# Runnlion/gaussian-splatting-slam

Hardware: AMD Instinct MI355X
Metric: train_iters_per_sec (higher is better)
Workload: dtype f32

## Files before the change

gaussian-splatting-slam_amd/csrc/ssim.hip:

```cpp
#include "gsr_common.h"

#define ST 32
#ifndef SSIM_STY
#define SSIM_STY 16
#endif
#define STY SSIM_STY
#define SR 5
#define SH (ST + 2 * SR)
#define SHY (STY + 2 * SR)
#define RPT (STY / 8)

struct SsimWindow { float g[11]; };

static SsimWindow make_window() {
  SsimWindow w;
  double v[11], s = 0.0;
  for (int i = 0; i < 11; i++) { v[i] = exp(-(double)((i - 5) * (i - 5)) / (2.0 * 1.5 * 1.5)); s += v[i]; }
  float f[11], fs = 0.f;
  for (int i = 0; i < 11; i++) { f[i] = (float)v[i]; fs += f[i]; }
  for (int i = 0; i < 11; i++) w.g[i] = f[i] / fs;
  (void)s;
  return w;
}


#define SSIM_XCDS 8
#define NTRIP ((SHY * SH + 255) / 256)
#ifndef SSIM_FWD_WAVES
#define SSIM_FWD_WAVES 5
#endif
struct SsimTile { int x0, y0; size_t plane; };
struct SsimWalk { long long first; int count; };
__device__ __forceinline__ SsimWalk ssim_walk(int gx, int gy, int planes, int tpw) {
  const long long n = (long long)gx * gy * planes;
  const long long per = (n + SSIM_XCDS - 1) / SSIM_XCDS;
  const long long strip = blockIdx.x % SSIM_XCDS, off = (long long)(blockIdx.x / SSIM_XCDS) * tpw;
  SsimWalk w;
  w.first = strip * per + off;
  long long last = strip * per + (off + tpw < per ? off + tpw : per);
  if (last > n) last = n;
  w.count = last > w.first ? (int)(last - w.first) : 0;
  return w;
}
__device__ __forceinline__ SsimTile ssim_tile_at(long long lin, int gx, int gy, int H, int W) {
  const int plane = (int)(lin / ((long long)gx * gy));
  const int rem = (int)(lin - (long long)plane * gx * gy);
  const int ty = rem / gx;
  SsimTile t;
  t.x0 = (rem - ty * gx) * ST;
  t.y0 = ty * STY;
  t.plane = (size_t)plane * H * W;
  return t;
}
static inline unsigned ssim_grid(int gx, int gy, int planes, int tpw) {
  const long long n = (long long)gx * gy * planes;
  const long long per = (n + SSIM_XCDS - 1) / SSIM_XCDS;
  return (unsigned)(((per + tpw - 1) / tpw) * SSIM_XCDS);
}
static inline int ssim_fwd_tpw(int gx, int gy, int planes) {
  static const int forced = getenv("GSR_SSIM_TPW") ? atoi(getenv("GSR_SSIM_TPW")) : 0;
  if (forced > 0) return forced;
  return (long long)gx * gy * planes >= 4096 ? 2 : 1;
}

__global__ __launch_bounds__(256) __attribute__((amdgpu_waves_per_eu(SSIM_FWD_WAVES, SSIM_FWD_WAVES))) void k_ssim_fwd(int H, int W, int planes, float C1, float C2, SsimWindow win,
                                                  const float* __restrict__ img1, const float* __restrict__ img2,
                                                  float* __restrict__ ssim_map, float* __restrict__ dm_dmu1,
                                                  float* __restrict__ dm_dsigma1_sq, float* __restrict__ dm_dsigma12,
                                                  float* __restrict__ partials, int tpw) {
  __shared__ float sx[SHY][SH + 1], sy[SHY][SH + 1];
  __shared__ float hm[5][SHY][ST + 1];
  __shared__ float wsum[4][2];
  const int tid0 = threadIdx.x;
  const int gxn = (W + ST - 1) / ST, gyn = (H + STY - 1) / STY;
  const SsimWalk walk = ssim_walk(gxn, gyn, planes, tpw);
  if (walk.count <= 0) return;
  float ra[NTRIP], rb[NTRIP];
  auto fetch = [&](long long lin, int tid) {
    const SsimTile t = ssim_tile_at(lin, gxn, gyn, H, W);
    int r = tid / SH, c = tid - r * SH;
#pragma unroll
    for (int k = 0; k < NTRIP; k++) {
      const int gy = t.y0 + r - SR, gx = t.x0 + c - SR;
      float a = 0.f, b = 0.f;
      if (tid + 256 * k < SHY * SH && gy >= 0 && gy < H && gx >= 0 && gx < W) {
        a = (img1 + t.plane)[gy * W + gx];
        b = (img2 + t.plane)[gy * W + gx];
      }
      ra[k] = a;
      rb[k] = b;
      r += 256 / SH; c += 256 % SH;
      if (c >= SH) { c -= SH; r++; }
    }
  };
  fetch(walk.first, tid0);
  for (int ti = 0; ti < walk.count; ti++) {
    int tid = tid0;
    asm volatile("" : "+v"(tid));
    const long long lin = walk.first + ti;
    const SsimTile tile = ssim_tile_at(lin, gxn, gyn, H, W);
    const int x0 = tile.x0, y0 = tile.y0;
    const size_t plane = tile.plane;
    {
      int r = tid / SH, c = tid - r * SH;
#pragma unroll
      for (int k = 0; k < NTRIP; k++) {
        if (tid + 256 * k < SHY * SH) { sx[r][c] = ra[k]; sy[r][c] = rb[k]; }
        r += 256 / SH; c += 256 % SH;
        if (c >= SH) { c -= SH; r++; }
      }
    }
    __syncthreads();
    if (ti > 0 && tid == 0 && partials) {
      partials[2 * (size_t)(lin - 1)] = (wsum[0][0] + wsum[1][0]) + (wsum[2][0] + wsum[3][0]);
      partials[2 * (size_t)(lin - 1) + 1] = (wsum[0][1] + wsum[1][1]) + (wsum[2][1] + wsum[3][1]);
    }
    if (ti + 1 < walk.count) fetch(lin + 1, tid);
    float acc_ssim = 0.f, acc_l1 = 0.f;
    for (int i = tid; i < SHY * (ST / 4); i += 256) {
      const int r = i / (ST / 4), c0 = (i - r * (ST / 4)) * 4;
      float xa[14], ya[14];
#pragma unroll
      for (int k = 0; k < 14; k++) { xa[k] = sx[r][c0 + k]; ya[k] = sy[r][c0 + k]; }
      if (r >= SR && r < SR + STY && y0 + r - SR < H) {
#pragma unroll
        for (int j = 0; j < 4; j++)
          if (x0 + c0 + j < W) acc_l1 += fabsf(xa[SR + j] - ya[SR + j]);
      }
#pragma unroll
      for (int j = 0; j < 4; j++) {
        float m1 = 0.f, m2 = 0.f, s11 = 0.f, s22 = 0.f, s12 = 0.f;
#pragma unroll
        for (int k = 0; k < 11; k++) {
          const float w = win.g[k], a = xa[j + k], b = ya[j + k];
          m1 += w * a; m2 += w * b; s11 += w * a * a; s22 += w * b * b; s12 += w * a * b;
        }
        hm[0][r][c0 + j] = m1; hm[1][r][c0 + j] = m2; hm[2][r][c0 + j] = s11; hm[3][r][c0 + j] = s22; hm[4][r][c0 + j] = s12;
      }
    }
    __syncthreads();
    {
      const int c = tid & (ST - 1), r0 = (tid / ST) * RPT;
      float col[5][RPT + 10];
#pragma unroll
      for (int q = 0; q < 5; q++)
#pragma unroll
        for (int k = 0; k < RPT + 10; k++) col[q][k] = hm[q][r0 + k][c];
#pragma unroll
      for (int j = 0; j < RPT; j++) {
        const int r = r0 + j;
        const int gy = y0 + r, gx = x0 + c;
        if (gy >= H || gx >= W) continue;
        float mu1 = 0.f, mu2 = 0.f, e11 = 0.f, e22 = 0.f, e12 = 0.f;
#pragma unroll
        for (int k = 0; k < 11; k++) {
          const float w = win.g[k];
          mu1 += w * col[0][j + k]; mu2 += w * col[1][j + k]; e11 += w * col[2][j + k];
          e22 += w * col[3][j + k]; e12 += w * col[4][j + k];
        }
        const float mu1_sq = mu1 * mu1, mu2_sq = mu2 * mu2, mu12 = mu1 * mu2;
        const float sigma1_sq = e11 - mu1_sq, sigma2_sq = e22 - mu2_sq, sigma12 = e12 - mu12;
        const float A = 2.f * mu12 + C1, B = 2.f * sigma12 + C2;
        const float Cc = mu1_sq + mu2_sq + C1, D = sigma1_sq + sigma2_sq + C2;
        const float rCc = __builtin_amdgcn_rcpf(Cc), rD = __builtin_amdgcn_rcpf(D);
        const float inv = rCc * rD;
        const float m = A * B * inv;
        const size_t o = plane + (size_t)gy * W + gx;
        if (ssim_map) ssim_map[o] = m;
        acc_ssim += m;
        if (dm_dmu1) {
          dm_dmu1[o] = 2.f * mu2 * (B - A) * inv - m * 2.f * mu1 * rCc + m * 2.f * mu1 * rD;
          dm_dsigma1_sq[o] = -m * rD;
          dm_dsigma12[o] = 2.f * A * inv;
        }
      }
    }
    if (partials) {
#pragma unroll
      for (int sft = 32; sft > 0; sft >>= 1) {
        acc_ssim += __shfl_down(acc_ssim, sft, 64);
        acc_l1 += __shfl_down(acc_l1, sft, 64);
      }
      if ((tid & 63) == 0) { wsum[tid >> 6][0] = acc_ssim; wsum[tid >> 6][1] = acc_l1; }
    }
  }
  if (partials) {
    __syncthreads();
    if (tid0 == 0) {
      const size_t lin = (size_t)(walk.first + walk.count - 1);
      partials[2 * lin] = (wsum[0][0] + wsum[1][0]) + (wsum[2][0] + wsum[3][0]);
      partials[2 * lin + 1] = (wsum[0][1] + wsum[1][1]) + (wsum[2][1] + wsum[3][1]);
    }
  }
}

__global__ __launch_bounds__(256) void k_ssim_bwd(int H, int W, int planes, SsimWindow win, const float* __restrict__ img1,
                                                  const float* __restrict__ img2, const float* __restrict__ dL_dmap,
                                                  float g_const, float g_l1, const float* __restrict__ upstream,
                                                  const float* __restrict__ dm_dmu1,
                                                  const float* __restrict__ dm_dsigma1_sq,
                                                  const float* __restrict__ dm_dsigma12, float* __restrict__ dL_dimg1) {
  __shared__ float sa[3][SHY][SH + 1];
  const int tid = threadIdx.x;
  const int gxn = (W + ST - 1) / ST, gyn = (H + STY - 1) / STY;
  const SsimWalk walk = ssim_walk(gxn, gyn, planes, 1);
  if (walk.count <= 0) return;
  const SsimTile tile = ssim_tile_at(walk.first, gxn, gyn, H, W);
  const int x0 = tile.x0, y0 = tile.y0;
  const size_t plane = tile.plane;
  if (upstream) {
    const float u = upstream[0];
    g_const *= u;
    g_l1 *= u;
  }
  int lr = tid / SH, lc = tid - lr * SH;
  for (int i = tid; i < SHY * SH; i += 256) {
    const int r = lr, c = lc;
    lr += 256 / SH; lc += 256 % SH;
    if (lc >= SH) { lc -= SH; lr++; }
    const int gy = y0 + r - SR, gx = x0 + c - SR;
    float a = 0.f, b = 0.f, d = 0.f;
    if (gy >= 0 && gy < H && gx >= 0 && gx < W) {
      const size_t o = plane + (size_t)gy * W + gx;
      const float g = dL_dmap ? dL_dmap[o] : g_const;
      a = g * dm_dmu1[o];
      b = g * dm_dsigma1_sq[o];
      d = g * dm_dsigma12[o];
    }
    sa[0][r][c] = a; sa[1][r][c] = b; sa[2][r][c] = d;
  }
  __syncthreads();
  for (int i = tid; i < SHY * (ST / 4); i += 256) {
    const int r = i / (ST / 4), c0 = (i - r * (ST / 4)) * 4;
    float v0[14], v1[14], v2[14];
#pragma unroll
    for (int k = 0; k < 14; k++) { v0[k] = sa[0][r][c0 + k]; v1[k] = sa[1][r][c0 + k]; v2[k] = sa[2][r][c0 + k]; }
    asm volatile("" ::: "memory");
    __builtin_amdgcn_wave_barrier();
#pragma unroll
    for (int j = 0; j < 4; j++) {
      float t0 = 0.f, t1 = 0.f, t2 = 0.f;
#pragma unroll
      for (int k = 0; k < 11; k++) {
        const float w = win.g[k];
        t0 += w * v0[j + k]; t1 += w * v1[j + k]; t2 += w * v2[j + k];
      }
      sa[0][r][c0 + j] = t0; sa[1][r][c0 + j] = t1; sa[2][r][c0 + j] = t2;
    }
  }
  __syncthreads();
  {
    const int c = tid & (ST - 1), r0 = (tid / ST) * RPT;
    float col[3][RPT + 10];
#pragma unroll
    for (int q = 0; q < 3; q++)
#pragma unroll
      for (int k = 0; k < RPT + 10; k++) col[q][k] = sa[q][r0 + k][c];
#pragma unroll
    for (int j = 0; j < RPT; j++) {
      const int gy = y0 + r0 + j, gx = x0 + c;
      if (gy >= H || gx >= W) continue;
      float t0 = 0.f, t1 = 0.f, t2 = 0.f;
#pragma unroll
      for (int k = 0; k < 11; k++) {
        const float w = win.g[k];
        t0 += w * col[0][j + k]; t1 += w * col[1][j + k]; t2 += w * col[2][j + k];
      }
      const size_t o = plane + (size_t)gy * W + gx;
      const float x = img1[o], y = img2[o];
      float out = t0 + 2.f * x * t1 + y * t2;
      if (!dL_dmap) out += g_l1 * ((x > y) ? 1.f : ((x < y) ? -1.f : 0.f));
      dL_dimg1[o] = out;
    }
  }
}

extern "C" {

int gsr_fused_ssim_forward(int32_t planes, int32_t H, int32_t W, float C1, float C2, const float* img1,
                           const float* img2, float* ssim_map, float* dm_dmu1, float* dm_dsigma1_sq,
                           float* dm_dsigma12, void* stream) {
  if (planes < 0 || H <= 0 || W <= 0 || !img1 || !img2 || !ssim_map ||
      ((dm_dmu1 != nullptr) != (dm_dsigma1_sq != nullptr)) || ((dm_dmu1 != nullptr) != (dm_dsigma12 != nullptr))) {
    gsr_set_error("fused_ssim_forward: bad arguments");
    return GSR_ERR_INVALID_ARGUMENT;
  }
  if (planes == 0) return 0;
  static const SsimWindow win = make_window();
  hipStream_t st = (hipStream_t)stream;
  dim3 grid((W + ST - 1) / ST, (H + STY - 1) / STY, planes);
  const int tpw = ssim_fwd_tpw(grid.x, grid.y, planes);
  GSR_LAUNCH("ssim_fwd", k_ssim_fwd, dim3(ssim_grid(grid.x, grid.y, planes, tpw)), dim3(256), 0, st, H, W, planes, C1, C2, win, img1, img2,
             ssim_map, dm_dmu1, dm_dsigma1_sq, dm_dsigma12, (float*)nullptr, tpw);
  return gsr_launch_status("ssim forward launch");
}

int64_t gsr_fused_loss_blocks(int32_t planes, int32_t H, int32_t W) {
  return (int64_t)((W + ST - 1) / ST) * ((H + STY - 1) / STY) * planes;
}

#define LOSS_FIN_THREADS 1024
__global__ __launch_bounds__(LOSS_FIN_THREADS) void k_loss_finalize(const float* __restrict__ partials, long long nblk,
                                                                    float lambda, float inv_n, float* __restrict__ loss) {
  __shared__ float red[2][LOSS_FIN_THREADS / 64];
  const float2* pairs = reinterpret_cast<const float2*>(partials);
  float a = 0.f, b = 0.f;
  long long i = threadIdx.x;
  for (; i + 3 * LOSS_FIN_THREADS < nblk; i += 4 * LOSS_FIN_THREADS) {
    const float2 v0 = pairs[i], v1 = pairs[i + LOSS_FIN_THREADS], v2 = pairs[i + 2 * LOSS_FIN_THREADS],
                 v3 = pairs[i + 3 * LOSS_FIN_THREADS];
    a += v0.x; b += v0.y;
    a += v1.x; b += v1.y;
    a += v2.x; b += v2.y;
    a += v3.x; b += v3.y;
  }
  for (; i < nblk; i += LOSS_FIN_THREADS) {
    const float2 v = pairs[i];
    a += v.x;
    b += v.y;
  }
#pragma unroll
  for (int sft = 32; sft > 0; sft >>= 1) {
    a += __shfl_down(a, sft, 64);
    b += __shfl_down(b, sft, 64);
  }
  if ((threadIdx.x & 63) == 0) { red[0][threadIdx.x >> 6] = a; red[1][threadIdx.x >> 6] = b; }
  __syncthreads();
  if (threadIdx.x < 64) {
    a = threadIdx.x < LOSS_FIN_THREADS / 64 ? red[0][threadIdx.x] : 0.f;
    b = threadIdx.x < LOSS_FIN_THREADS / 64 ? red[1][threadIdx.x] : 0.f;
#pragma unroll
    for (int sft = LOSS_FIN_THREADS / 128; sft > 0; sft >>= 1) {
      a += __shfl_down(a, sft, 64);
      b += __shfl_down(b, sft, 64);
    }
    if (threadIdx.x == 0) loss[0] = (1.0f - lambda) * (b * inv_n) + lambda * (1.0f - a * inv_n);
  }
}

int gsr_fused_l1_ssim_forward(int32_t planes, int32_t H, int32_t W, float C1, float C2, float lambda_dssim,
                              const float* img1, const float* img2, float* dm_dmu1, float* dm_dsigma1_sq,
                              float* dm_dsigma12, float* partials, float* loss, void* stream) {
  if (planes <= 0 || H <= 0 || W <= 0 || !img1 || !img2 || !dm_dmu1 || !dm_dsigma1_sq || !dm_dsigma12 || !partials ||
      !loss) {
    gsr_set_error("fused_l1_ssim_forward: bad arguments");
    return GSR_ERR_INVALID_ARGUMENT;
  }
  static const SsimWindow win = make_window();
  hipStream_t st = (hipStream_t)stream;
  dim3 grid((W + ST - 1) / ST, (H + STY - 1) / STY, planes);
  const int tpw = ssim_fwd_tpw(grid.x, grid.y, planes);
  GSR_LAUNCH("loss_fwd", k_ssim_fwd, dim3(ssim_grid(grid.x, grid.y, planes, tpw)), dim3(256), 0, st, H, W, planes, C1, C2, win, img1, img2,
             (float*)nullptr, dm_dmu1, dm_dsigma1_sq, dm_dsigma12, partials, tpw);
  const long long nblk = (long long)grid.x * grid.y * grid.z;
  const float inv_n = 1.0f / ((float)planes * (float)H * (float)W);
  GSR_LAUNCH("loss_finalize", k_loss_finalize, dim3(1), dim3(LOSS_FIN_THREADS), 0, st, (const float*)partials, nblk, lambda_dssim,
             inv_n, loss);
  return gsr_launch_status("fused loss forward launch");
}

int gsr_fused_l1_ssim_backward(int32_t planes, int32_t H, int32_t W, float lambda_dssim, const float* img1,
                               const float* img2, const float* upstream, const float* dm_dmu1,
                               const float* dm_dsigma1_sq, const float* dm_dsigma12, float* dL_dimg1, void* stream) {
  if (planes <= 0 || H <= 0 || W <= 0 || !img1 || !img2 || !dm_dmu1 || !dm_dsigma1_sq || !dm_dsigma12 || !dL_dimg1) {
    gsr_set_error("fused_l1_ssim_backward: bad arguments");
    return GSR_ERR_INVALID_ARGUMENT;
  }
  static const SsimWindow win = make_window();
  hipStream_t st = (hipStream_t)stream;
  dim3 grid((W + ST - 1) / ST, (H + STY - 1) / STY, planes);
  const float inv_n = 1.0f / ((float)planes * (float)H * (float)W);
  GSR_LAUNCH("loss_bwd", k_ssim_bwd, dim3(ssim_grid(grid.x, grid.y, planes, 1)), dim3(256), 0, st, H, W, planes, win, img1, img2, (const float*)nullptr,
             -lambda_dssim * inv_n, (1.0f - lambda_dssim) * inv_n, upstream, dm_dmu1, dm_dsigma1_sq, dm_dsigma12,
             dL_dimg1);
  return gsr_launch_status("fused loss backward launch");
}

int gsr_fused_ssim_backward(int32_t planes, int32_t H, int32_t W, const float* img1, const float* img2,
                            const float* dL_dmap, const float* dm_dmu1, const float* dm_dsigma1_sq,
                            const float* dm_dsigma12, float* dL_dimg1, void* stream) {
  if (planes < 0 || H <= 0 || W <= 0 || !img1 || !img2 || !dL_dmap || !dm_dmu1 || !dm_dsigma1_sq || !dm_dsigma12 ||
      !dL_dimg1) {
    gsr_set_error("fused_ssim_backward: bad arguments");
    return GSR_ERR_INVALID_ARGUMENT;
  }
  if (planes == 0) return 0;
  static const SsimWindow win = make_window();
  hipStream_t st = (hipStream_t)stream;
  dim3 grid((W + ST - 1) / ST, (H + STY - 1) / STY, planes);
  GSR_LAUNCH("ssim_bwd", k_ssim_bwd, dim3(ssim_grid(grid.x, grid.y, planes, 1)), dim3(256), 0, st, H, W, planes, win, img1, img2, dL_dmap, 0.f, 0.f,
             (const float*)nullptr, dm_dmu1, dm_dsigma1_sq, dm_dsigma12, dL_dimg1);
  return gsr_launch_status("ssim backward launch");
}

#define L1_BLOCKS 1024
__global__ __launch_bounds__(256) void k_l1_partial(const float* __restrict__ a, const float* __restrict__ b,
                                                    const float* __restrict__ mask, long long n, float* __restrict__ partials) {
  __shared__ float red[256];
  float acc = 0.f;
  const long long n4 = n >> 2;
  const float4* a4 = reinterpret_cast<const float4*>(a);
  const float4* b4 = reinterpret_cast<const float4*>(b);
  const float4* m4 = reinterpret_cast<const float4*>(mask);
  for (long long i = (long long)blockIdx.x * 256 + threadIdx.x; i < n4; i += (long long)gridDim.x * 256) {
    const float4 x = a4[i], y = b4[i];
    const float4 m = mask ? m4[i] : make_float4(1.f, 1.f, 1.f, 1.f);
    acc += (fabsf((x.x - y.x) * m.x) + fabsf((x.y - y.y) * m.y)) + (fabsf((x.z - y.z) * m.z) + fabsf((x.w - y.w) * m.w));
  }
  if (blockIdx.x == 0 && (long long)threadIdx.x < (n & 3)) {
    const long long i = 4 * n4 + threadIdx.x;
    acc += fabsf((a[i] - b[i]) * (mask ? mask[i] : 1.f));
  }
  red[threadIdx.x] = acc;
  __syncthreads();
  for (int sft = 128; sft > 0; sft >>= 1) {
    if ((int)threadIdx.x < sft) red[threadIdx.x] += red[threadIdx.x + sft];
    __syncthreads();
  }
  if (threadIdx.x == 0) partials[blockIdx.x] = red[0];
}

__global__ __launch_bounds__(L1_BLOCKS) void k_l1_finalize(const float* __restrict__ partials, int nblk, float scale,
                                                           float* __restrict__ out) {
  __shared__ float red[L1_BLOCKS];
  red[threadIdx.x] = (int)threadIdx.x < nblk ? partials[threadIdx.x] : 0.f;
  __syncthreads();
  for (int sft = L1_BLOCKS / 2; sft > 0; sft >>= 1) {
    if ((int)threadIdx.x < sft) red[threadIdx.x] += red[threadIdx.x + sft];
    __syncthreads();
  }
  if (threadIdx.x == 0) out[0] = red[0] * scale;
}

__global__ __launch_bounds__(256) void k_l1_bwd(const float* __restrict__ a, const float* __restrict__ b,
                                                const float* __restrict__ mask, long long n, const float* __restrict__ upstream,
                                                float scale, float* __restrict__ grad) {
  const float g = (upstream ? upstream[0] : 1.0f) * scale;
  for (long long i = (long long)blockIdx.x * 256 + threadIdx.x; i < n; i += (long long)gridDim.x * 256) {
    const float m = mask ? mask[i] : 1.f;
    const float d = (a[i] - b[i]) * m;
    grad[i] = d > 0.f ? g * m : (d < 0.f ? -g * m : 0.f);
  }
}

int32_t gsr_l1_mean_blocks(void) { return L1_BLOCKS; }

int gsr_l1_mean_forward(int64_t n, float weight, const float* a, const float* b, const float* mask, float* partials, float* out,
                        void* stream) {
  if (n <= 0 || !a || !b || !partials || !out || (((uintptr_t)a | (uintptr_t)b | (uintptr_t)mask) & 15)) {
    gsr_set_error("l1_mean_forward: bad arguments");
    return GSR_ERR_INVALID_ARGUMENT;
  }
  hipStream_t st = (hipStream_t)stream;
  const int nblk = (int)min((long long)L1_BLOCKS, (long long)((n / 4 + 255) / 256 > 0 ? (n / 4 + 255) / 256 : 1));
  GSR_LAUNCH("l1_partial", k_l1_partial, dim3(nblk), dim3(256), 0, st, a, b, mask, (long long)n, partials);
  GSR_LAUNCH("l1_finalize", k_l1_finalize, dim3(1), dim3(L1_BLOCKS), 0, st, (const float*)partials, nblk, weight / (float)n, out);
  return gsr_launch_status("l1 mean forward launch");
}

int gsr_l1_mean_backward(int64_t n, float weight, const float* a, const float* b, const float* mask, const float* upstream,
                         float* grad, void* stream) {
  if (n <= 0 || !a || !b || !grad) {
    gsr_set_error("l1_mean_backward: bad arguments");
    return GSR_ERR_INVALID_ARGUMENT;
  }
  const int nblk = (int)min((long long)4096, (long long)((n + 255) / 256));
  GSR_LAUNCH("l1_bwd", k_l1_bwd, dim3(nblk), dim3(256), 0, (hipStream_t)stream, a, b, mask, (long long)n, upstream, weight / (float)n, grad);
  return gsr_launch_status("l1 mean backward launch");
}

}
```

Baseline: 799.8.

## Rewrite SSIM forward as per-wave column strips with a rolling register ring

Replaces the block-tiled SSIM forward kernel, which used shared-memory tiles and two block-wide barriers per tile, with a per-wavefront design. Each wave owns a 64-wide column strip covering a segment of 24 rows. It streams rows through a small LDS row buffer using only wave barriers, computes the horizontal pass per row, and keeps the last 11 horizontal results in a register ring for the vertical pass. This removes block synchronisation and halo recomputation between tiles, at the cost of more vertical halo overhead per segment, higher register pressure from the ring, and partials counted per wave-unit instead of per tile.

```diff
diff --git a/gaussian-splatting-slam_amd/csrc/ssim.hip b/gaussian-splatting-slam_amd/csrc/ssim.hip
--- a/gaussian-splatting-slam_amd/csrc/ssim.hip
+++ b/gaussian-splatting-slam_amd/csrc/ssim.hip
@@ -1,34 +1,171 @@
 #include "gsr_common.h"
 
+#define SR 5
+#define SW 64
+#define SBUF (SW + 2 * SR + 2)
+#define SSIM_WAVES 4
+#define SSIM_XCDS 8
+
+struct SsimWindow { float g[11]; };
+
+static SsimWindow make_window() {
+  SsimWindow w;
+  double v[11];
+  for (int i = 0; i < 11; i++) v[i] = exp(-(double)((i - 5) * (i - 5)) / (2.0 * 1.5 * 1.5));
+  float f[11], fs = 0.f;
+  for (int i = 0; i < 11; i++) { f[i] = (float)v[i]; fs += f[i]; }
+  for (int i = 0; i < 11; i++) w.g[i] = f[i] / fs;
+  return w;
+}
+
+static inline int ssim_seg_len(int H, int W, int planes) {
+  static const int forced = getenv("GSR_SSIM_SEG") ? atoi(getenv("GSR_SSIM_SEG")) : 0;
+  if (forced > 0) return forced;
+  return 24;
+}
+
+static inline long long ssim_units(int H, int W, int planes, int L) {
+  return (long long)((W + SW - 1) / SW) * ((H + L - 1) / L) * planes;
+}
+static inline long long ssim_per_xcd(long long n) {
+  const long long per = (n + SSIM_XCDS - 1) / SSIM_XCDS;
+  return (per + SSIM_WAVES - 1) / SSIM_WAVES * SSIM_WAVES;
+}
+static inline unsigned ssim_grid(int H, int W, int planes, int L) {
+  return (unsigned)(ssim_per_xcd(ssim_units(H, W, planes, L)) / SSIM_WAVES * SSIM_XCDS);
+}
+struct SsimUnit { long long u; int x0, y0, nout; size_t plane; };
+__device__ __forceinline__ bool ssim_unit_of_wave(int H, int W, int planes, int L, SsimUnit& t) {
+  const int wv = __builtin_amdgcn_readfirstlane((int)(threadIdx.x >> 6));
+  const int nsx = (W + SW - 1) / SW, nsy = (H + L - 1) / L;
+  const long long n = (long long)nsx * nsy * planes;
+  long long per = (n + SSIM_XCDS - 1) / SSIM_XCDS;
+  per = (per + SSIM_WAVES - 1) / SSIM_WAVES * SSIM_WAVES;
+  const long long band = blockIdx.x % SSIM_XCDS;
+  const long long u = band * per + (long long)(blockIdx.x / SSIM_XCDS) * SSIM_WAVES + wv;
+  const long long end = (band + 1) * per < n ? (band + 1) * per : n;
+  if (u >= end) return false;
+  const int pl = (int)(u / ((long long)nsx * nsy));
+  const int rem = (int)(u - (long long)pl * nsx * nsy);
+  const int sy = rem / nsx;
+  t.u = u;
+  t.x0 = (rem - sy * nsx) * SW;
+  t.y0 = sy * L;
+  t.nout = H - t.y0 < L ? H - t.y0 : L;
+  t.plane = (size_t)pl * H * W;
+  return true;
+}
+__device__ __forceinline__ void ssim_lds_fence() {
+  asm volatile("" ::: "memory");
+  __builtin_amdgcn_wave_barrier();
+  asm volatile("" ::: "memory");
+}
+
+__global__ __launch_bounds__(64 * SSIM_WAVES) void k_ssim_fwd(int H, int W, int planes, float C1, float C2, SsimWindow win,
+                                                  const float* __restrict__ img1, const float* __restrict__ img2,
+                                                  float* __restrict__ ssim_map, float* __restrict__ dm_dmu1,
+                                                  float* __restrict__ dm_dsigma1_sq, float* __restrict__ dm_dsigma12,
+                                                  float* __restrict__ partials, int L) {
+  __shared__ float rowbuf[SSIM_WAVES][2][SBUF];
+  SsimUnit t;
+  if (!ssim_unit_of_wave(H, W, planes, L, t)) return;
+  const int lane = threadIdx.x & 63;
+  float* bx = rowbuf[__builtin_amdgcn_readfirstlane((int)(threadIdx.x >> 6))][0];
+  float* by = bx + SBUF;
+  const float* p1 = img1 + t.plane;
+  const float* p2 = img2 + t.plane;
+  const int y0 = t.y0, nout = t.nout, nrows = nout + 2 * SR;
+  const int gx = t.x0 + lane;
+  const int hx = t.x0 + (lane < SR ? lane - SR : SW - SR + lane);
+  const int hi = lane < SR ? lane : SW + lane;
+  const bool main_ok = gx < W, halo_ok = lane < 2 * SR && hx >= 0 && hx < W;
+  float a0, b0, a1, b1;
+  auto fetch = [&](int gy) {
+    a0 = 0.f; b0 = 0.f; a1 = 0.f; b1 = 0.f;
+    if (gy >= 0 && gy < H) {
+      if (main_ok) { a0 = p1[gy * W + gx]; b0 = p2[gy * W + gx]; }
+      if (halo_ok) { a1 = p1[gy * W + hx]; b1 = p2[gy * W + hx]; }
+    }
+  };
+  fetch(y0 - SR);
+  float ring[5][11];
+  float acc_ssim = 0.f, acc_l1 = 0.f;
+  for (int j0 = 0; j0 < nrows; j0 += 11) {
+#pragma unroll
+    for (int p = 0; p < 11; p++) {
+      const int j = j0 + p;
+      if (j >= nrows) break;
+      const int gy = y0 - SR + j;
+      ssim_lds_fence();
+      bx[SR + lane] = a0; by[SR + lane] = b0;
+      if (lane < 2 * SR) { bx[hi] = a1; by[hi] = b1; }
+      ssim_lds_fence();
+      if (j + 1 < nrows) fetch(gy + 1);
+      float xa[11], ya[11];
+#pragma unroll
+      for (int k = 0; k < 11; k++) { xa[k] = bx[lane + k]; ya[k] = by[lane + k]; }
+      if (gy >= y0 && gy < y0 + nout) acc_l1 += fabsf(xa[SR] - ya[SR]);
+      {
+        float m1 = 0.f, m2 = 0.f, s11 = 0.f, s22 = 0.f, s12 = 0.f;
+#pragma unroll
+        for (int k = 0; k < 11; k++) {
+          const float w = win.g[k], a = xa[k], b = ya[k];
+          m1 += w * a; m2 += w * b; s11 += w * a * a; s22 += w * b * b; s12 += w * a * b;
+        }
+        ring[0][p] = m1; ring[1][p] = m2; ring[2][p] = s11; ring[3][p] = s22; ring[4][p] = s12;
+      }
+      if (j0 == 0 && p < 2 * SR) continue;
+      const int oy = gy - SR;
+      if (!main_ok) continue;
+      float mu1 = 0.f, mu2 = 0.f, e11 = 0.f, e22 = 0.f, e12 = 0.f;
+#pragma unroll
+      for (int k = 0; k < 11; k++) {
+        const float w = win.g[k];
+        const int s = (p + 1 + k) % 11;
+        mu1 += w * ring[0][s]; mu2 += w * ring[1][s]; e11 += w * ring[2][s];
+        e22 += w * ring[3][s]; e12 += w * ring[4][s];
+      }
+      float A, B, inv, m, rCc, rD;
+      {
+#pragma clang fp contract(off)
+        const float mu2_sq = mu2 * mu2, mu12 = mu1 * mu2;
+        const float sigma1_sq = __builtin_fmaf(-mu1, mu1, e11), sigma2_sq = __builtin_fmaf(-mu2, mu2, e22);
+        const float sigma12 = __builtin_fmaf(-mu1, mu2, e12);
+        A = __builtin_fmaf(2.f, mu12, C1);
+        B = __builtin_fmaf(2.f, sigma12, C2);
+        const float Cc = __builtin_fmaf(mu1, mu1, mu2_sq) + C1, D = (sigma1_sq + sigma2_sq) + C2;
+        rCc = __builtin_amdgcn_rcpf(Cc);
+        rD = __builtin_amdgcn_rcpf(D);
+        inv = rCc * rD;
+        m = (A * B) * inv;
+      }
+      const size_t o = t.plane + (size_t)oy * W + gx;
+      if (ssim_map) ssim_map[o] = m;
+      acc_ssim += m;
+      if (dm_dmu1) {
+#pragma clang fp contract(off)
+        const float u = ((mu2 + mu2) * (B - A)), v = (m + m) * mu1;
+        dm_dmu1[o] = __builtin_fmaf(rD, v, __builtin_fmaf(inv, u, -(rCc * v)));
+        dm_dsigma1_sq[o] = -m * rD;
+        dm_dsigma12[o] = (A + A) * inv;
+      }
+    }
+  }
+  if (partials) {
+#pragma unroll
+    for (int sft = 32; sft > 0; sft >>= 1) {
+      acc_ssim += __shfl_down(acc_ssim, sft, 64);
+      acc_l1 += __shfl_down(acc_l1, sft, 64);
+    }
+    if (lane == 0) { partials[2 * (size_t)t.u] = acc_ssim; partials[2 * (size_t)t.u + 1] = acc_l1; }
+  }
+}
+
 #define ST 32
-#ifndef SSIM_STY
-#define SSIM_STY 16
-#endif
-#define STY SSIM_STY
-#define SR 5
+#define STY 16
 #define SH (ST + 2 * SR)
 #define SHY (STY + 2 * SR)
 #define RPT (STY / 8)
-
-struct SsimWindow { float g[11]; };
-
-static SsimWindow make_window() {
-  SsimWindow w;
-  double v[11], s = 0.0;
-  for (int i = 0; i < 11; i++) { v[i] = exp(-(double)((i - 5) * (i - 5)) / (2.0 * 1.5 * 1.5)); s += v[i]; }
-  float f[11], fs = 0.f;
-  for (int i = 0; i < 11; i++) { f[i] = (float)v[i]; fs += f[i]; }
-  for (int i = 0; i < 11; i++) w.g[i] = f[i] / fs;
-  (void)s;
-  return w;
-}
-
-
-#define SSIM_XCDS 8
-#define NTRIP ((SHY * SH + 255) / 256)
-#ifndef SSIM_FWD_WAVES
-#define SSIM_FWD_WAVES 5
-#endif
 struct SsimTile { int x0, y0; size_t plane; };
 struct SsimWalk { long long first; int count; };
 __device__ __forceinline__ SsimWalk ssim_walk(int gx, int gy, int planes, int tpw) {
@@ -52,146 +189,9 @@
   t.plane = (size_t)plane * H * W;
   return t;
 }
-static inline unsigned ssim_grid(int gx, int gy, int planes, int tpw) {
+static inline unsigned ssim_tile_grid(int gx, int gy, int planes) {
   const long long n = (long long)gx * gy * planes;
-  const long long per = (n + SSIM_XCDS - 1) / SSIM_XCDS;
-  return (unsigned)(((per + tpw - 1) / tpw) * SSIM_XCDS);
-}
-static inline int ssim_fwd_tpw(int gx, int gy, int planes) {
-  static const int forced = getenv("GSR_SSIM_TPW") ? atoi(getenv("GSR_SSIM_TPW")) : 0;
-  if (forced > 0) return forced;
-  return (long long)gx * gy * planes >= 4096 ? 2 : 1;
-}
-
-__global__ __launch_bounds__(256) __attribute__((amdgpu_waves_per_eu(SSIM_FWD_WAVES, SSIM_FWD_WAVES))) void k_ssim_fwd(int H, int W, int planes, float C1, float C2, SsimWindow win,
-                                                  const float* __restrict__ img1, const float* __restrict__ img2,
-                                                  float* __restrict__ ssim_map, float* __restrict__ dm_dmu1,
-                                                  float* __restrict__ dm_dsigma1_sq, float* __restrict__ dm_dsigma12,
-                                                  float* __restrict__ partials, int tpw) {
-  __shared__ float sx[SHY][SH + 1], sy[SHY][SH + 1];
-  __shared__ float hm[5][SHY][ST + 1];
-  __shared__ float wsum[4][2];
-  const int tid0 = threadIdx.x;
-  const int gxn = (W + ST - 1) / ST, gyn = (H + STY - 1) / STY;
-  const SsimWalk walk = ssim_walk(gxn, gyn, planes, tpw);
-  if (walk.count <= 0) return;
-  float ra[NTRIP], rb[NTRIP];
-  auto fetch = [&](long long lin, int tid) {
-    const SsimTile t = ssim_tile_at(lin, gxn, gyn, H, W);
-    int r = tid / SH, c = tid - r * SH;
-#pragma unroll
-    for (int k = 0; k < NTRIP; k++) {
-      const int gy = t.y0 + r - SR, gx = t.x0 + c - SR;
-      float a = 0.f, b = 0.f;
-      if (tid + 256 * k < SHY * SH && gy >= 0 && gy < H && gx >= 0 && gx < W) {
-        a = (img1 + t.plane)[gy * W + gx];
-        b = (img2 + t.plane)[gy * W + gx];
-      }
-      ra[k] = a;
-      rb[k] = b;
-      r += 256 / SH; c += 256 % SH;
-      if (c >= SH) { c -= SH; r++; }
-    }
-  };
-  fetch(walk.first, tid0);
-  for (int ti = 0; ti < walk.count; ti++) {
-    int tid = tid0;
-    asm volatile("" : "+v"(tid));
-    const long long lin = walk.first + ti;
-    const SsimTile tile = ssim_tile_at(lin, gxn, gyn, H, W);
-    const int x0 = tile.x0, y0 = tile.y0;
-    const size_t plane = tile.plane;
-    {
-      int r = tid / SH, c = tid - r * SH;
-#pragma unroll
-      for (int k = 0; k < NTRIP; k++) {
-        if (tid + 256 * k < SHY * SH) { sx[r][c] = ra[k]; sy[r][c] = rb[k]; }
-        r += 256 / SH; c += 256 % SH;
-        if (c >= SH) { c -= SH; r++; }
-      }
-    }
-    __syncthreads();
-    if (ti > 0 && tid == 0 && partials) {
-      partials[2 * (size_t)(lin - 1)] = (wsum[0][0] + wsum[1][0]) + (wsum[2][0] + wsum[3][0]);
-      partials[2 * (size_t)(lin - 1) + 1] = (wsum[0][1] + wsum[1][1]) + (wsum[2][1] + wsum[3][1]);
-    }
-    if (ti + 1 < walk.count) fetch(lin + 1, tid);
-    float acc_ssim = 0.f, acc_l1 = 0.f;
-    for (int i = tid; i < SHY * (ST / 4); i += 256) {
-      const int r = i / (ST / 4), c0 = (i - r * (ST / 4)) * 4;
-      float xa[14], ya[14];
-#pragma unroll
-      for (int k = 0; k < 14; k++) { xa[k] = sx[r][c0 + k]; ya[k] = sy[r][c0 + k]; }
-      if (r >= SR && r < SR + STY && y0 + r - SR < H) {
-#pragma unroll
-        for (int j = 0; j < 4; j++)
-          if (x0 + c0 + j < W) acc_l1 += fabsf(xa[SR + j] - ya[SR + j]);
-      }
-#pragma unroll
-      for (int j = 0; j < 4; j++) {
-        float m1 = 0.f, m2 = 0.f, s11 = 0.f, s22 = 0.f, s12 = 0.f;
-#pragma unroll
-        for (int k = 0; k < 11; k++) {
-          const float w = win.g[k], a = xa[j + k], b = ya[j + k];
-          m1 += w * a; m2 += w * b; s11 += w * a * a; s22 += w * b * b; s12 += w * a * b;
-        }
-        hm[0][r][c0 + j] = m1; hm[1][r][c0 + j] = m2; hm[2][r][c0 + j] = s11; hm[3][r][c0 + j] = s22; hm[4][r][c0 + j] = s12;
-      }
-    }
-    __syncthreads();
-    {
-      const int c = tid & (ST - 1), r0 = (tid / ST) * RPT;
-      float col[5][RPT + 10];
-#pragma unroll
-      for (int q = 0; q < 5; q++)
-#pragma unroll
-        for (int k = 0; k < RPT + 10; k++) col[q][k] = hm[q][r0 + k][c];
-#pragma unroll
-      for (int j = 0; j < RPT; j++) {
-        const int r = r0 + j;
-        const int gy = y0 + r, gx = x0 + c;
-        if (gy >= H || gx >= W) continue;
-        float mu1 = 0.f, mu2 = 0.f, e11 = 0.f, e22 = 0.f, e12 = 0.f;
-#pragma unroll
-        for (int k = 0; k < 11; k++) {
-          const float w = win.g[k];
-          mu1 += w * col[0][j + k]; mu2 += w * col[1][j + k]; e11 += w * col[2][j + k];
-          e22 += w * col[3][j + k]; e12 += w * col[4][j + k];
-        }
-        const float mu1_sq = mu1 * mu1, mu2_sq = mu2 * mu2, mu12 = mu1 * mu2;
-        const float sigma1_sq = e11 - mu1_sq, sigma2_sq = e22 - mu2_sq, sigma12 = e12 - mu12;
-        const float A = 2.f * mu12 + C1, B = 2.f * sigma12 + C2;
-        const float Cc = mu1_sq + mu2_sq + C1, D = sigma1_sq + sigma2_sq + C2;
-        const float rCc = __builtin_amdgcn_rcpf(Cc), rD = __builtin_amdgcn_rcpf(D);
-        const float inv = rCc * rD;
-        const float m = A * B * inv;
-        const size_t o = plane + (size_t)gy * W + gx;
-        if (ssim_map) ssim_map[o] = m;
-        acc_ssim += m;
-        if (dm_dmu1) {
-          dm_dmu1[o] = 2.f * mu2 * (B - A) * inv - m * 2.f * mu1 * rCc + m * 2.f * mu1 * rD;
-          dm_dsigma1_sq[o] = -m * rD;
-          dm_dsigma12[o] = 2.f * A * inv;
-        }
-      }
-    }
-    if (partials) {
-#pragma unroll
-      for (int sft = 32; sft > 0; sft >>= 1) {
-        acc_ssim += __shfl_down(acc_ssim, sft, 64);
-        acc_l1 += __shfl_down(acc_l1, sft, 64);
-      }
-      if ((tid & 63) == 0) { wsum[tid >> 6][0] = acc_ssim; wsum[tid >> 6][1] = acc_l1; }
-    }
-  }
-  if (partials) {
-    __syncthreads();
-    if (tid0 == 0) {
-      const size_t lin = (size_t)(walk.first + walk.count - 1);
-      partials[2 * lin] = (wsum[0][0] + wsum[1][0]) + (wsum[2][0] + wsum[3][0]);
-      partials[2 * lin + 1] = (wsum[0][1] + wsum[1][1]) + (wsum[2][1] + wsum[3][1]);
-    }
-  }
+  return (unsigned)((n + SSIM_XCDS - 1) / SSIM_XCDS * SSIM_XCDS);
 }
 
 __global__ __launch_bounds__(256) void k_ssim_bwd(int H, int W, int planes, SsimWindow win, const float* __restrict__ img1,
@@ -288,15 +288,15 @@
   if (planes == 0) return 0;
   static const SsimWindow win = make_window();
   hipStream_t st = (hipStream_t)stream;
-  dim3 grid((W + ST - 1) / ST, (H + STY - 1) / STY, planes);
-  const int tpw = ssim_fwd_tpw(grid.x, grid.y, planes);
-  GSR_LAUNCH("ssim_fwd", k_ssim_fwd, dim3(ssim_grid(grid.x, grid.y, planes, tpw)), dim3(256), 0, st, H, W, planes, C1, C2, win, img1, img2,
-             ssim_map, dm_dmu1, dm_dsigma1_sq, dm_dsigma12, (float*)nullptr, tpw);
+  const int L = ssim_seg_len(H, W, planes);
+  GSR_LAUNCH("ssim_fwd", k_ssim_fwd, dim3(ssim_grid(H, W, planes, L)), dim3(64 * SSIM_WAVES), 0, st, H, W, planes, C1, C2, win, img1, img2,
+             ssim_map, dm_dmu1, dm_dsigma1_sq, dm_dsigma12, (float*)nullptr, L);
   return gsr_launch_status("ssim forward launch");
 }
 
 int64_t gsr_fused_loss_blocks(int32_t planes, int32_t H, int32_t W) {
-  return (int64_t)((W + ST - 1) / ST) * ((H + STY - 1) / STY) * planes;
+  if (planes <= 0 || H <= 0 || W <= 0) return 0;
+  return (int64_t)ssim_units(H, W, planes, ssim_seg_len(H, W, planes));
 }
 
 #define LOSS_FIN_THREADS 1024
@@ -348,11 +348,10 @@
   }
   static const SsimWindow win = make_window();
   hipStream_t st = (hipStream_t)stream;
-  dim3 grid((W + ST - 1) / ST, (H + STY - 1) / STY, planes);
-  const int tpw = ssim_fwd_tpw(grid.x, grid.y, planes);
-  GSR_LAUNCH("loss_fwd", k_ssim_fwd, dim3(ssim_grid(grid.x, grid.y, planes, tpw)), dim3(256), 0, st, H, W, planes, C1, C2, win, img1, img2,
-             (float*)nullptr, dm_dmu1, dm_dsigma1_sq, dm_dsigma12, partials, tpw);
-  const long long nblk = (long long)grid.x * grid.y * grid.z;
+  const int L = ssim_seg_len(H, W, planes);
+  GSR_LAUNCH("loss_fwd", k_ssim_fwd, dim3(ssim_grid(H, W, planes, L)), dim3(64 * SSIM_WAVES), 0, st, H, W, planes, C1, C2, win, img1, img2,
+             (float*)nullptr, dm_dmu1, dm_dsigma1_sq, dm_dsigma12, partials, L);
+  const long long nblk = ssim_units(H, W, planes, L);
   const float inv_n = 1.0f / ((float)planes * (float)H * (float)W);
   GSR_LAUNCH("loss_finalize", k_loss_finalize, dim3(1), dim3(LOSS_FIN_THREADS), 0, st, (const float*)partials, nblk, lambda_dssim,
              inv_n, loss);
@@ -370,7 +369,7 @@
   hipStream_t st = (hipStream_t)stream;
   dim3 grid((W + ST - 1) / ST, (H + STY - 1) / STY, planes);
   const float inv_n = 1.0f / ((float)planes * (float)H * (float)W);
-  GSR_LAUNCH("loss_bwd", k_ssim_bwd, dim3(ssim_grid(grid.x, grid.y, planes, 1)), dim3(256), 0, st, H, W, planes, win, img1, img2, (const float*)nullptr,
+  GSR_LAUNCH("loss_bwd", k_ssim_bwd, dim3(ssim_tile_grid(grid.x, grid.y, planes)), dim3(256), 0, st, H, W, planes, win, img1, img2, (const float*)nullptr,
              -lambda_dssim * inv_n, (1.0f - lambda_dssim) * inv_n, upstream, dm_dmu1, dm_dsigma1_sq, dm_dsigma12,
              dL_dimg1);
   return gsr_launch_status("fused loss backward launch");
@@ -388,7 +387,7 @@
   static const SsimWindow win = make_window();
   hipStream_t st = (hipStream_t)stream;
   dim3 grid((W + ST - 1) / ST, (H + STY - 1) / STY, planes);
-  GSR_LAUNCH("ssim_bwd", k_ssim_bwd, dim3(ssim_grid(grid.x, grid.y, planes, 1)), dim3(256), 0, st, H, W, planes, win, img1, img2, dL_dmap, 0.f, 0.f,
+  GSR_LAUNCH("ssim_bwd", k_ssim_bwd, dim3(ssim_tile_grid(grid.x, grid.y, planes)), dim3(256), 0, st, H, W, planes, win, img1, img2, dL_dmap, 0.f, 0.f,
              (const float*)nullptr, dm_dmu1, dm_dsigma1_sq, dm_dsigma12, dL_dimg1);
   return gsr_launch_status("ssim backward launch");
 }
```

Measured after the change: 811.6 (median of 6 runs). 1.5% higher.
